# Lightning-AI/lit-llama

Hardware: NVIDIA H100
Metric: LLaMA-7B gptq.int4 decode tokens/sec (higher is better)
Workload: dtype bf16

## Files before the change

### __graft_entry__.py

```python
import os
import subprocess
import sys

ROOT = os.path.dirname(os.path.abspath(__file__))
PKG = os.path.join(ROOT, "lit-llama_b200")
CSRC = os.path.join(PKG, "csrc")
LIB = os.path.join(PKG, "libb200llama.so")
DIAG_LIB = os.path.join(ROOT, "tools", "libb200diag.so")
OBJ_DIR = os.path.join(ROOT, "build", "obj")
SOURCES = ["api.cu", "q_generic.cu", "elementwise.cu", "attention.cu", "q4_tc.cu", "q4_gemv.cu", "q4_gemv_batch.cu",
           "q8_gemv.cu", "q8_gemm.cu", "sampling.cu", "decode_mega.cu", "q4_gemm.cu", "tp_allreduce.cu", "lora.cu",
           "nll.cu", "w8_gemv_batch.cu", "q8_gemv_batch.cu"]
DIAG_SOURCES = ["microbench.cu"]
ARCH = ["-gencode", "arch=compute_90a,code=sm_90a"]
NVCC_FLAGS = ARCH + ["-O3", "-lineinfo", "-std=c++17", "-Xcompiler", "-fPIC"]


def _headers():
    return [os.path.join(CSRC, f) for f in os.listdir(CSRC) if f.endswith((".cuh", ".h"))] + \
           [os.path.join(ROOT, "include", f) for f in os.listdir(os.path.join(ROOT, "include"))]


def _compile(nvcc: str, src: str, force: bool) -> str:
    obj = os.path.join(OBJ_DIR, os.path.splitext(src)[0] + ".o")
    path = os.path.join(CSRC, src)
    if not force and os.path.exists(obj):
        t = os.path.getmtime(obj)
        if all(os.path.getmtime(d) <= t for d in [path] + _headers()):
            return obj
    cmd = [nvcc] + NVCC_FLAGS + ["-c", path, "-o", obj]
    print("[build]", " ".join(cmd), file=sys.stderr)
    subprocess.run(cmd, check=True)
    return obj


def _link(nvcc: str, objs, out: str) -> None:
    if os.path.exists(out) and all(os.path.getmtime(o) <= os.path.getmtime(out) for o in objs):
        return
    cmd = [nvcc, "-shared"] + ARCH + list(objs) + ["-o", out]
    print("[build]", " ".join(cmd), file=sys.stderr)
    subprocess.run(cmd, check=True)


def build(force: bool = False) -> None:
    from concurrent.futures import ThreadPoolExecutor

    nvcc = os.environ.get("NVCC", "/usr/local/cuda/bin/nvcc")
    os.makedirs(OBJ_DIR, exist_ok=True)
    with ThreadPoolExecutor(max_workers=min(8, os.cpu_count() or 1)) as ex:
        objs = list(ex.map(lambda s: _compile(nvcc, s, force), SOURCES + DIAG_SOURCES))
    _link(nvcc, objs[:len(SOURCES)], LIB)
    _link(nvcc, objs[len(SOURCES):], DIAG_LIB)
    _install_reference()
    if ROOT not in sys.path:
        sys.path.insert(0, ROOT)
    import lit_llama_b200
    from lit_llama_b200 import _lib

    assert _lib.lib().b2l_version() >= 100


def _install_reference(src: str = os.environ.get("LIT_LLAMA_DIR", "/root/reference")) -> None:
    import shutil
    import tempfile

    dst = os.path.join(ROOT, "oracle", "_ref")
    if os.path.isdir(os.path.join(dst, "lit_llama")) or not os.path.isfile(os.path.join(src, "pyproject.toml")):
        return
    tmp = tempfile.mkdtemp(prefix="b2l_ref_")
    try:
        work = os.path.join(tmp, "reference")
        shutil.copytree(src, work, ignore=shutil.ignore_patterns(".git", "tests", "howto"))
        cmd = [sys.executable, "-m", "pip", "install", "--no-index", "--no-build-isolation", "--no-deps", "--quiet",
               "--target", dst, work]
        print("[build]", " ".join(cmd), file=sys.stderr)
        subprocess.run(cmd, check=False)
    finally:
        shutil.rmtree(tmp, ignore_errors=True)


def smoke() -> None:
    if ROOT not in sys.path:
        sys.path.insert(0, ROOT)
    import torch

    import lit_llama_b200 as P
    from lit_llama_b200.utils import quantization
    from oracle import llama_oracle as O

    assert torch.cuda.is_available(), "smoke() needs a GPU"
    dev = torch.device("cuda", 0)
    cfg = dict(block_size=64, vocab_size=96, n_layer=2, n_head=4, n_embd=128)
    sd = O.synth_state_dict(cfg["n_layer"], cfg["n_head"], cfg["n_embd"], cfg["vocab_size"], "gptq.int4",
                            dtype=torch.bfloat16, seed=1234)
    prev = torch.get_default_dtype()
    torch.set_default_dtype(torch.bfloat16)
    try:
        with torch.device(dev), quantization("gptq.int4"):
            model = P.LLaMA(P.LLaMAConfig(**cfg))
    finally:
        torch.set_default_dtype(prev)
    model.load_state_dict(sd)
    model.eval()
    oracle = O.OracleLLaMA.from_state_dict(sd, cfg["n_layer"], cfg["n_head"], cfg["block_size"], "gptq.int4")
    prompt = torch.tensor([3, 17, 40, 41, 2, 77, 5], dtype=torch.int32)
    S = 16
    with torch.no_grad():
        got = [model(prompt.view(1, -1).to(dev), S, torch.arange(7, device=dev))]
        want = [oracle.forward(prompt.view(1, -1).long(), S, torch.arange(7))]
        for i, t in enumerate([11, 5, 90, 33]):
            got.append(model(torch.tensor([[t]], dtype=torch.int32, device=dev), S, torch.tensor([7 + i], device=dev)))
            want.append(oracle.forward(torch.tensor([[t]]), S, torch.tensor([7 + i])))
    torch.cuda.synchronize()
    for g, w in zip(got, want):
        torch.testing.assert_close(g.float().cpu(), w.float(), rtol=1e-3, atol=5e-3)
    print("smoke ok: tiny gptq.int4 prefill + 4 decode steps match the oracle", file=sys.stderr)


if __name__ == "__main__":
    build(force="--force" in sys.argv)
    if "--smoke" in sys.argv:
        smoke()
```

### include/b2l_diag.h

```cpp
#ifndef B2L_DIAG_H_
#define B2L_DIAG_H_
#include "b2l.h"
#ifdef __cplusplus
extern "C" {
#endif

const char* b2l_diag_last_error(void);

int b2l_debug_grid_flag(void* out, void* counter, int ctas_per_sm, int rounds, b2l_stream_t stream);

int b2l_debug_hmma_rate(void* out, int warps, int chains, int iters, int with_unpack, b2l_stream_t stream);

int b2l_debug_imma_rate(void* out, int warps, int chains, int iters, int n_alu, b2l_stream_t stream);

int b2l_debug_consumer_rate(void* out, int warps, int iters, int mode, int n_ctas, b2l_stream_t stream);

#ifdef __cplusplus
}
#endif
#endif
```

### lit-llama_b200/csrc/sampling.cu

```cuda
#include "b2l_common.cuh"

namespace b2l {

constexpr int SAMP_THREADS = 1024;

__device__ __forceinline__ uint32_t bf16_key(uint16_t b) {
  return (b & 0x8000u) ? (uint32_t)(uint16_t)~b : (uint32_t)(b | 0x8000u);
}

__device__ __forceinline__ void hist_add(int* hist, uint32_t bin, bool valid) {
  const uint32_t key = valid ? bin : 0xFFFFFFFFu;
  const uint32_t peers = __match_any_sync(0xffffffffu, key);
  if (valid && (threadIdx.x & 31) == __ffs(peers) - 1) atomicAdd(&hist[bin], __popc(peers));
}

__device__ __forceinline__ void find_bin(const int* hist, int want, int* sel_bin, int* sel_rank) {
  const int lane = threadIdx.x & 31;
  int c[8], s = 0;
#pragma unroll
  for (int j = 0; j < 8; ++j) { c[j] = hist[lane * 8 + j]; s += c[j]; }
  int incl = s;
#pragma unroll
  for (int o = 1; o < 32; o <<= 1) {
    const int t = __shfl_down_sync(0xffffffffu, incl, o);
    if (lane + o < 32) incl += t;
  }
  const int above = incl - s;
  if (above < want && want <= above + s) {
    int cum = above;
#pragma unroll
    for (int j = 7; j >= 0; --j) {
      if (cum + c[j] >= want) { *sel_bin = lane * 8 + j; *sel_rank = want - cum; break; }
      cum += c[j];
    }
  }
}

__device__ __forceinline__ float bits_f(uint32_t bits16) { return __uint_as_float(bits16 << 16); }

__device__ __forceinline__ uint4 load8(const __nv_bfloat16* p, int i, bool vec) {
  if (vec) return reinterpret_cast<const uint4*>(p)[i];
  const uint16_t* s = reinterpret_cast<const uint16_t*>(p) + 8 * i;
  return make_uint4(s[0] | ((uint32_t)s[1] << 16), s[2] | ((uint32_t)s[3] << 16), s[4] | ((uint32_t)s[5] << 16),
                    s[6] | ((uint32_t)s[7] << 16));
}

__global__ void __launch_bounds__(SAMP_THREADS)
    topk_softmax_kernel(const __nv_bfloat16* __restrict__ logits, long long ld, float inv_temperature, int top_k,
                        __nv_bfloat16* __restrict__ probs, const __nv_bfloat16* __restrict__ noise,
                        long long* __restrict__ token, int V) {
  extern __shared__ __align__(16) uint8_t ssm[];
  {
    const size_t row = blockIdx.x;
    logits += row * (size_t)ld;
    if (noise != nullptr) noise += row * (size_t)V;
    if (probs != nullptr) probs += row * (size_t)V;
    if (token != nullptr) token += row;
  }
  const bool vec = ((reinterpret_cast<uintptr_t>(logits) | reinterpret_cast<uintptr_t>(noise)) & 15) == 0;
  const int Vp = (V + 7) & ~7;
  uint16_t* sv = reinterpret_cast<uint16_t*>(ssm);
  uint16_t* sq = sv + Vp;
  __shared__ int hist[256];
  __shared__ int sel_hi, sel_rank, sel_lo;
  __shared__ float red[32];
  __shared__ int red_i[32];
  const int tid = threadIdx.x, lane = tid & 31, warp = tid >> 5;
  const bool select = top_k > 0 && top_k < V;
  const int nvec = V / 8;
  constexpr int PRE = 4;

  uint4 lpre[PRE], npre[PRE];
#pragma unroll
  for (int r = 0; r < PRE; ++r) {
    const int i = r * SAMP_THREADS + tid;
    lpre[r] = make_uint4(0, 0, 0, 0);
    npre[r] = make_uint4(0, 0, 0, 0);
    if (i < nvec) {
      lpre[r] = load8(logits, i, vec);
      if (noise != nullptr) npre[r] = load8(noise, i, vec);
    }
  }

  if (tid < 256) hist[tid] = 0;
  __syncthreads();
  float lmax = -INFINITY;
  const int rounds = (nvec + SAMP_THREADS - 1) / SAMP_THREADS;
#pragma unroll 1
  for (int r0 = 0; r0 < rounds; r0 += PRE) {
#pragma unroll
    for (int rr = 0; rr < PRE; ++rr) {
      const int r = r0 + rr;
      if (r >= rounds) break;
      const int i = r * SAMP_THREADS + tid;
      const bool valid = i < nvec;
      uint4 v = lpre[rr];
      if (r0 > 0) { v = make_uint4(0, 0, 0, 0); if (valid) v = load8(logits, i, vec); }
      const uint32_t w[4] = {v.x, v.y, v.z, v.w};
      uint32_t o[4];
#pragma unroll
      for (int q = 0; q < 4; ++q) {
        const float a = rbf(__uint_as_float(w[q] << 16) * inv_temperature);
        const float b = rbf(__uint_as_float(w[q] & 0xffff0000u) * inv_temperature);
        const uint32_t ab = __float_as_uint(a) >> 16, bb = __float_as_uint(b) >> 16;
        o[q] = ab | (bb << 16);
        if (valid) lmax = fmaxf(lmax, fmaxf(a, b));
        if (select) {
          hist_add(hist, bf16_key((uint16_t)ab) >> 8, valid);
          hist_add(hist, bf16_key((uint16_t)bb) >> 8, valid);
        }
      }
      if (valid) {
        reinterpret_cast<uint4*>(sv)[i] = make_uint4(o[0], o[1], o[2], o[3]);
        if (noise != nullptr) {
          uint4 n = npre[rr];
          if (r0 > 0) n = load8(noise, i, vec);
          reinterpret_cast<uint4*>(sq)[i] = n;
        }
      }
    }
  }
  {
    const int i = nvec * 8 + tid;
    const bool valid = i < V;
    uint16_t bits = 0xff80;
    if (valid) {
      const float sc = rbf(bf2f(logits[i]) * inv_temperature);
      bits = (uint16_t)(__float_as_uint(sc) >> 16);
      lmax = fmaxf(lmax, sc);
    }
    if (i < Vp) {
      sv[i] = bits;
      if (noise != nullptr) sq[i] = valid ? *reinterpret_cast<const uint16_t*>(noise + i) : (uint16_t)0x3f80;
    }
    if (select) hist_add(hist, bf16_key(bits) >> 8, valid);
  }
  lmax = warp_max(lmax);
  if (lane == 0) red[warp] = lmax;
  __syncthreads();
  float gmax = red[lane];
  gmax = warp_max(gmax);

  const int nvp = Vp / 8;
  uint32_t thr_key = 0;
  if (select) {
    if (warp == 0) find_bin(hist, top_k, &sel_hi, &sel_rank);
    __syncthreads();
    const int hi = sel_hi, rank = sel_rank;
    __syncthreads();
    if (tid < 256) hist[tid] = 0;
    __syncthreads();
    for (int base = 0; base < nvp; base += SAMP_THREADS) {
      const int i = base + tid;
      uint4 v = make_uint4(0, 0, 0, 0);
      if (i < nvp) v = reinterpret_cast<const uint4*>(sv)[i];
      const uint32_t w[4] = {v.x, v.y, v.z, v.w};
#pragma unroll
      for (int q = 0; q < 4; ++q) {
#pragma unroll
        for (int hf = 0; hf < 2; ++hf) {
          const uint32_t key = bf16_key((uint16_t)(hf ? (w[q] >> 16) : (w[q] & 0xffffu)));
          const bool hit = i < nvp && (int)(key >> 8) == hi && (8 * i + 2 * q + hf) < V;
          if (__any_sync(0xffffffffu, hit)) hist_add(hist, key & 0xFF, hit);
        }
      }
    }
    __syncthreads();
    if (warp == 0) { int dummy; find_bin(hist, rank, &sel_lo, &dummy); }
    __syncthreads();
    thr_key = ((uint32_t)hi << 8) | (uint32_t)sel_lo;
  }

  float sum = 0.f;
  for (int base = 0; base < nvp; base += SAMP_THREADS) {
    const int i = base + tid;
    if (i < nvp) {
      const uint4 v = reinterpret_cast<const uint4*>(sv)[i];
      const uint32_t w[4] = {v.x, v.y, v.z, v.w};
      bool any = false;
#pragma unroll
      for (int q = 0; q < 4; ++q)
        any = any || bf16_key((uint16_t)(w[q] & 0xffffu)) >= thr_key || bf16_key((uint16_t)(w[q] >> 16)) >= thr_key;
      if (any) {
#pragma unroll
        for (int q = 0; q < 4; ++q) {
          const uint32_t lo = w[q] & 0xffffu, hi2 = w[q] >> 16;
          if (bf16_key((uint16_t)lo) >= thr_key && lo != 0xff80u) sum += expf(bits_f(lo) - gmax);
          if (bf16_key((uint16_t)hi2) >= thr_key && hi2 != 0xff80u) sum += expf(bits_f(hi2) - gmax);
        }
      }
    }
  }
  sum = warp_sum(sum);
  __syncthreads();
  if (lane == 0) red[warp] = sum;
  __syncthreads();
  float total = red[lane];
  total = warp_sum(total);

  float best = -INFINITY;
  int best_i = 0x7fffffff;
  for (int base = 0; base < nvp; base += SAMP_THREADS) {
    const int i = base + tid;
    if (i < nvp) {
      const uint4 v = reinterpret_cast<const uint4*>(sv)[i];
      uint4 n = make_uint4(0, 0, 0, 0);
      if (noise != nullptr) n = reinterpret_cast<const uint4*>(sq)[i];
      const uint32_t w[4] = {v.x, v.y, v.z, v.w};
      const uint32_t nw[4] = {n.x, n.y, n.z, n.w};
      uint32_t o[4] = {0u, 0u, 0u, 0u};
      bool any = false;
#pragma unroll
      for (int q = 0; q < 4; ++q)
        any = any || bf16_key((uint16_t)(w[q] & 0xffffu)) >= thr_key || bf16_key((uint16_t)(w[q] >> 16)) >= thr_key;
#pragma unroll
      for (int q = 0; q < 4; ++q) {
        if (!any) break;
        uint32_t pb2[2];
#pragma unroll
        for (int hf = 0; hf < 2; ++hf) {
          const uint32_t bits = hf ? (w[q] >> 16) : (w[q] & 0xffffu);
          const bool kept = bf16_key((uint16_t)bits) >= thr_key && bits != 0xff80u;
          const float pv = kept ? expf(bits_f(bits) - gmax) / total : 0.f;
          const float pr = rbf(pv);
          pb2[hf] = __float_as_uint(pr) >> 16;
          if (noise != nullptr) {
            const int idx = 8 * i + 2 * q + hf;
            const float r = rbf(pr / bits_f(hf ? (nw[q] >> 16) : (nw[q] & 0xffffu)));
            if (idx < V && (r > best || (r == best && idx < best_i))) { best = r; best_i = idx; }
          }
        }
        o[q] = pb2[0] | (pb2[1] << 16);
      }
      if (probs != nullptr) {
        if (8 * i + 8 <= V && (reinterpret_cast<uintptr_t>(probs) & 15) == 0) {
          reinterpret_cast<uint4*>(probs)[i] = make_uint4(o[0], o[1], o[2], o[3]);
        } else {
#pragma unroll
          for (int e = 0; e < 8; ++e)
            if (8 * i + e < V) reinterpret_cast<uint16_t*>(probs)[8 * i + e] = (uint16_t)(o[e >> 1] >> (16 * (e & 1)));
        }
      }
    }
  }
  if (noise != nullptr) {
#pragma unroll
    for (int o = 16; o > 0; o >>= 1) {
      const float ob = __shfl_xor_sync(0xffffffffu, best, o);
      const int oi = __shfl_xor_sync(0xffffffffu, best_i, o);
      if (ob > best || (ob == best && oi < best_i)) { best = ob; best_i = oi; }
    }
    __syncthreads();
    if (lane == 0) { red[warp] = best; red_i[warp] = best_i; }
    __syncthreads();
    if (warp == 0) {
      best = red[lane]; best_i = red_i[lane];
#pragma unroll
      for (int o = 16; o > 0; o >>= 1) {
        const float ob = __shfl_xor_sync(0xffffffffu, best, o);
        const int oi = __shfl_xor_sync(0xffffffffu, best_i, o);
        if (ob > best || (ob == best && oi < best_i)) { best = ob; best_i = oi; }
      }
      if (lane == 0) *token = (long long)best_i;
    }
  }
}

}

using namespace b2l;

static int launch_topk(const void* logits, long long ld, float temperature, int top_k, void* probs, const void* noise, void* token,
                       int B, int V, b2l_stream_t stream, const char* who) {
  B2L_CHECK_ARG(logits && V > 0 && temperature > 0.f && top_k >= 0, "%s: bad argument", who);
  B2L_CHECK_ARG(ld == 0 || ld >= V, "%s: ld = %lld: 0 (every row reads the same logits) or at least V = %d", who, ld, V);
  B2L_CHECK_ARG(((uintptr_t)logits % 16) == 0, "%s: logits must be 16-byte aligned", who);
  B2L_CHECK_ARG(noise == nullptr || ((uintptr_t)noise % 16) == 0, "%s: noise must be 16-byte aligned", who);
  const size_t Vp = ((size_t)V + 7) & ~(size_t)7;
  const size_t smem = Vp * 2 * (noise != nullptr ? 2 : 1);
  B2L_CHECK_SUPPORTED(smem <= 200 * 1024, "%s: vocabulary %d too large for one CTA", who, V);
  static DynSmemCache smem_cache;
  if (smem > 48 * 1024)
    if (int rc = ensure_dyn_smem(topk_softmax_kernel, smem, smem_cache)) return rc;
  topk_softmax_kernel<<<B, SAMP_THREADS, smem, (cudaStream_t)stream>>>((const __nv_bfloat16*)logits, ld, 1.0f / temperature, top_k,
                                                                      (__nv_bfloat16*)probs, (const __nv_bfloat16*)noise,
                                                                      (long long*)token, V);
  B2L_LAUNCH_CHECK("topk_softmax_kernel");
  return 0;
}

extern "C" int b2l_topk_softmax(const void* logits, float temperature, int top_k, void* probs, int V, b2l_stream_t stream) {
  B2L_CHECK_ARG(probs != nullptr, "b2l_topk_softmax: null probs");
  return launch_topk(logits, V, temperature, top_k, probs, nullptr, nullptr, 1, V, stream, "b2l_topk_softmax");
}

extern "C" int b2l_topk_softmax_sample(const void* logits, float temperature, int top_k, const void* noise, void* probs,
                                       int64_t* token, int V, b2l_stream_t stream) {
  B2L_CHECK_ARG(noise != nullptr && token != nullptr, "b2l_topk_softmax_sample: null noise / token");
  return launch_topk(logits, V, temperature, top_k, probs, noise, token, 1, V, stream, "b2l_topk_softmax_sample");
}

static int check_rows(const void* logits, int B, int V, float temperature, int top_k, const char* who) {
  B2L_CHECK_ARG(logits != nullptr, "%s: null logits", who);
  B2L_CHECK_ARG(B >= 1, "%s: B = %d rows, at least 1", who, B);
  B2L_CHECK_ARG(V > 0, "%s: V = %d, at least 1", who, V);
  B2L_CHECK_ARG(temperature > 0.f, "%s: temperature %g, must be positive", who, (double)temperature);
  B2L_CHECK_ARG(top_k >= 0, "%s: top_k = %d, 0 (no filter) or positive", who, top_k);
  return 0;
}

extern "C" int b2l_topk_softmax_rows(const void* logits, int64_t ld, float temperature, int top_k, void* probs, int B, int V,
                                     b2l_stream_t stream) {
  const char* who = "b2l_topk_softmax_rows";
  if (int rc = check_rows(logits, B, V, temperature, top_k, who)) return rc;
  B2L_CHECK_ARG(probs != nullptr, "%s: null probs", who);
  return launch_topk(logits, ld, temperature, top_k, probs, nullptr, nullptr, B, V, stream, who);
}

extern "C" int b2l_topk_softmax_sample_rows(const void* logits, int64_t ld, float temperature, int top_k, const void* noise,
                                            void* probs, int64_t* tokens, int B, int V, b2l_stream_t stream) {
  const char* who = "b2l_topk_softmax_sample_rows";
  if (int rc = check_rows(logits, B, V, temperature, top_k, who)) return rc;
  B2L_CHECK_ARG(noise != nullptr, "%s: null noise", who);
  B2L_CHECK_ARG(tokens != nullptr, "%s: null tokens", who);
  return launch_topk(logits, ld, temperature, top_k, probs, noise, tokens, B, V, stream, who);
}
```

Before: 596.4.

## Split top-k softmax sampling across an 8-CTA thread-block cluster with DSMEM exchange

```diff
diff --git a/__graft_entry__.py b/__graft_entry__.py
--- a/__graft_entry__.py
+++ b/__graft_entry__.py
@@ -11,7 +11,7 @@
 SOURCES = ["api.cu", "q_generic.cu", "elementwise.cu", "attention.cu", "q4_tc.cu", "q4_gemv.cu", "q4_gemv_batch.cu",
            "q8_gemv.cu", "q8_gemm.cu", "sampling.cu", "decode_mega.cu", "q4_gemm.cu", "tp_allreduce.cu", "lora.cu",
            "nll.cu", "w8_gemv_batch.cu", "q8_gemv_batch.cu"]
-DIAG_SOURCES = ["microbench.cu"]
+DIAG_SOURCES = ["microbench.cu", "sampling_cta.cu"]
 ARCH = ["-gencode", "arch=compute_90a,code=sm_90a"]
 NVCC_FLAGS = ARCH + ["-O3", "-lineinfo", "-std=c++17", "-Xcompiler", "-fPIC"]
 
diff --git a/include/b2l_diag.h b/include/b2l_diag.h
--- a/include/b2l_diag.h
+++ b/include/b2l_diag.h
@@ -15,6 +15,9 @@
 
 int b2l_debug_consumer_rate(void* out, int warps, int iters, int mode, int n_ctas, b2l_stream_t stream);
 
+int b2l_debug_topk_softmax_cta(const void* logits, int64_t ld, float temperature, int top_k, const void* noise, void* probs,
+                               int64_t* tokens, int B, int V, b2l_stream_t stream);
+
 #ifdef __cplusplus
 }
 #endif
diff --git a/lit-llama_b200/csrc/sampling.cu b/lit-llama_b200/csrc/sampling.cu
--- a/lit-llama_b200/csrc/sampling.cu
+++ b/lit-llama_b200/csrc/sampling.cu
@@ -1,57 +1,53 @@
-#include "b2l_common.cuh"
+#include <cooperative_groups.h>
+
+#include "sampling_common.cuh"
+
+namespace cg = cooperative_groups;
 
 namespace b2l {
 
-constexpr int SAMP_THREADS = 1024;
-
-__device__ __forceinline__ uint32_t bf16_key(uint16_t b) {
-  return (b & 0x8000u) ? (uint32_t)(uint16_t)~b : (uint32_t)(b | 0x8000u);
-}
-
-__device__ __forceinline__ void hist_add(int* hist, uint32_t bin, bool valid) {
-  const uint32_t key = valid ? bin : 0xFFFFFFFFu;
-  const uint32_t peers = __match_any_sync(0xffffffffu, key);
-  if (valid && (threadIdx.x & 31) == __ffs(peers) - 1) atomicAdd(&hist[bin], __popc(peers));
-}
-
-__device__ __forceinline__ void find_bin(const int* hist, int want, int* sel_bin, int* sel_rank) {
-  const int lane = threadIdx.x & 31;
-  int c[8], s = 0;
-#pragma unroll
-  for (int j = 0; j < 8; ++j) { c[j] = hist[lane * 8 + j]; s += c[j]; }
-  int incl = s;
-#pragma unroll
-  for (int o = 1; o < 32; o <<= 1) {
-    const int t = __shfl_down_sync(0xffffffffu, incl, o);
-    if (lane + o < 32) incl += t;
-  }
-  const int above = incl - s;
-  if (above < want && want <= above + s) {
-    int cum = above;
-#pragma unroll
-    for (int j = 7; j >= 0; --j) {
-      if (cum + c[j] >= want) { *sel_bin = lane * 8 + j; *sel_rank = want - cum; break; }
-      cum += c[j];
-    }
-  }
-}
-
-__device__ __forceinline__ float bits_f(uint32_t bits16) { return __uint_as_float(bits16 << 16); }
-
-__device__ __forceinline__ uint4 load8(const __nv_bfloat16* p, int i, bool vec) {
-  if (vec) return reinterpret_cast<const uint4*>(p)[i];
-  const uint16_t* s = reinterpret_cast<const uint16_t*>(p) + 8 * i;
-  return make_uint4(s[0] | ((uint32_t)s[1] << 16), s[2] | ((uint32_t)s[3] << 16), s[4] | ((uint32_t)s[5] << 16),
-                    s[6] | ((uint32_t)s[7] << 16));
-}
-
-__global__ void __launch_bounds__(SAMP_THREADS)
-    topk_softmax_kernel(const __nv_bfloat16* __restrict__ logits, long long ld, float inv_temperature, int top_k,
-                        __nv_bfloat16* __restrict__ probs, const __nv_bfloat16* __restrict__ noise,
-                        long long* __restrict__ token, int V) {
+constexpr int SAMP_CLUSTER = 8;
+constexpr int SAMP_VT = SAMP_THREADS / SAMP_CLUSTER;
+constexpr int SAMP_CL_THREADS = 4 * SAMP_VT;
+constexpr int SAMP_CL_WARPS = SAMP_CL_THREADS / 32;
+static_assert(SAMP_VT % 32 == 0 && SAMP_CLUSTER * (SAMP_VT / 32) == 32, "the cluster holds the one-CTA kernel's 32 warps");
+static_assert(SAMP_VT / 32 == 4, "a CTA's warp sums are pushed as one 16-byte vector");
+constexpr int SAMP_HI_WORDS = 260;
+
+__device__ __forceinline__ uint32_t smem_u32(const void* p) { return (uint32_t)__cvta_generic_to_shared(p); }
+__device__ __forceinline__ uint32_t remote_u32(const void* local, int rank) {
+  uint32_t r;
+  asm volatile("mapa.shared::cluster.u32 %0, %1, %2;" : "=r"(r) : "r"(smem_u32(local)), "r"(rank));
+  return r;
+}
+__device__ __forceinline__ void st_async_v4(uint32_t dst, uint4 v, uint32_t bar) {
+  asm volatile("st.async.shared::cluster.mbarrier::complete_tx::bytes.v4.b32 [%0], {%1, %2, %3, %4}, [%5];" ::"r"(dst),
+               "r"(v.x), "r"(v.y), "r"(v.z), "r"(v.w), "r"(bar) : "memory");
+}
+__device__ __forceinline__ void st_async_v2(uint32_t dst, uint32_t a, uint32_t b, uint32_t bar) {
+  asm volatile("st.async.shared::cluster.mbarrier::complete_tx::bytes.v2.b32 [%0], {%1, %2}, [%3];" ::"r"(dst), "r"(a), "r"(b),
+               "r"(bar) : "memory");
+}
+__device__ __forceinline__ void mbar_init_expect(uint64_t* bar, uint32_t bytes) {
+  asm volatile("mbarrier.init.shared::cta.b64 [%0], 1;" ::"r"(smem_u32(bar)) : "memory");
+  asm volatile("mbarrier.arrive.expect_tx.shared::cta.b64 _, [%0], %1;" ::"r"(smem_u32(bar)), "r"(bytes) : "memory");
+}
+__device__ __forceinline__ void mbar_wait0(uint64_t* bar) {
+  asm volatile(
+      "{\n\t.reg .pred P1;\n\tLAB_WAIT:\n\t"
+      "mbarrier.try_wait.parity.shared::cta.b64 P1, [%0], 0;\n\t"
+      "@P1 bra DONE;\n\tbra LAB_WAIT;\n\tDONE:\n\t}" ::"r"(smem_u32(bar)) : "memory");
+}
+
+__global__ void __launch_bounds__(SAMP_CL_THREADS)
+    topk_softmax_cluster_kernel(const __nv_bfloat16* __restrict__ logits, long long ld, float inv_temperature, int top_k,
+                                __nv_bfloat16* __restrict__ probs, const __nv_bfloat16* __restrict__ noise,
+                                long long* __restrict__ token, int V) {
   extern __shared__ __align__(16) uint8_t ssm[];
+  cg::cluster_group cluster = cg::this_cluster();
+  const int rank = (int)cluster.block_rank();
   {
-    const size_t row = blockIdx.x;
+    const size_t row = blockIdx.x / SAMP_CLUSTER;
     logits += row * (size_t)ld;
     if (noise != nullptr) noise += row * (size_t)V;
     if (probs != nullptr) probs += row * (size_t)V;
@@ -59,40 +55,64 @@
   }
   const bool vec = ((reinterpret_cast<uintptr_t>(logits) | reinterpret_cast<uintptr_t>(noise)) & 15) == 0;
   const int Vp = (V + 7) & ~7;
+  const int nvec = V / 8;
+  const int nvp = Vp / 8;
+  const int rounds = (nvp + SAMP_THREADS - 1) / SAMP_THREADS;
+  const int nslot = rounds * SAMP_VT;
+  auto vec_of = [rank](int s) { return (s / SAMP_VT) * SAMP_THREADS + rank * SAMP_VT + s % SAMP_VT; };
   uint16_t* sv = reinterpret_cast<uint16_t*>(ssm);
-  uint16_t* sq = sv + Vp;
-  __shared__ int hist[256];
+  uint16_t* sq = sv + nslot * 8;
+  __shared__ __align__(16) int hist_hi[256];
+  __shared__ __align__(16) int hist_lo[256];
+  __shared__ __align__(16) int rx_hi[SAMP_CLUSTER][SAMP_HI_WORDS];
+  __shared__ __align__(16) int rx_lo[SAMP_CLUSTER][256];
+  __shared__ __align__(16) float wsum[32];
+  __shared__ __align__(16) float red_sum[SAMP_VT / 32];
+  __shared__ __align__(8) uint32_t cl_best[SAMP_CLUSTER][2];
+  __shared__ __align__(8) uint64_t mbar[4];
+  __shared__ int ghist[256];
   __shared__ int sel_hi, sel_rank, sel_lo;
-  __shared__ float red[32];
-  __shared__ int red_i[32];
+  __shared__ float cta_max, gmax_s;
+  __shared__ float red[SAMP_CL_WARPS];
+  __shared__ int red_i[SAMP_CL_WARPS];
   const int tid = threadIdx.x, lane = tid & 31, warp = tid >> 5;
   const bool select = top_k > 0 && top_k < V;
-  const int nvec = V / 8;
-  constexpr int PRE = 4;
+  if (tid == 0) {
+    mbar_init_expect(&mbar[0], SAMP_CLUSTER * (select ? SAMP_HI_WORDS * 4 : 16));
+    mbar_init_expect(&mbar[1], select ? SAMP_CLUSTER * 1024 : 0);
+    mbar_init_expect(&mbar[2], SAMP_CLUSTER * 16);
+    mbar_init_expect(&mbar[3], rank == 0 && noise != nullptr ? SAMP_CLUSTER * 8 : 0);
+    asm volatile("fence.mbarrier_init.release.cluster;" ::: "memory");
+  }
+  asm volatile("barrier.cluster.arrive.relaxed.aligned;" ::: "memory");
+  constexpr int PRE = 2;
 
   uint4 lpre[PRE], npre[PRE];
 #pragma unroll
   for (int r = 0; r < PRE; ++r) {
-    const int i = r * SAMP_THREADS + tid;
+    const int s = r * SAMP_CL_THREADS + tid;
+    const int i = vec_of(s);
     lpre[r] = make_uint4(0, 0, 0, 0);
     npre[r] = make_uint4(0, 0, 0, 0);
-    if (i < nvec) {
+    if (s < nslot && i < nvec) {
       lpre[r] = load8(logits, i, vec);
       if (noise != nullptr) npre[r] = load8(noise, i, vec);
     }
   }
 
-  if (tid < 256) hist[tid] = 0;
+  if (tid < 256) { hist_hi[tid] = 0; hist_lo[tid] = 0; }
   __syncthreads();
   float lmax = -INFINITY;
-  const int rounds = (nvec + SAMP_THREADS - 1) / SAMP_THREADS;
+  const int iters = (nslot + SAMP_CL_THREADS - 1) / SAMP_CL_THREADS;
 #pragma unroll 1
-  for (int r0 = 0; r0 < rounds; r0 += PRE) {
+  for (int r0 = 0; r0 < iters; r0 += PRE) {
 #pragma unroll
     for (int rr = 0; rr < PRE; ++rr) {
       const int r = r0 + rr;
-      if (r >= rounds) break;
-      const int i = r * SAMP_THREADS + tid;
+      if (r >= iters) break;
+      const int s = r * SAMP_CL_THREADS + tid;
+      if (s >= nslot) break;
+      const int i = vec_of(s);
       const bool valid = i < nvec;
       uint4 v = lpre[rr];
       if (r0 > 0) { v = make_uint4(0, 0, 0, 0); if (valid) v = load8(logits, i, vec); }
@@ -106,54 +126,79 @@
         o[q] = ab | (bb << 16);
         if (valid) lmax = fmaxf(lmax, fmaxf(a, b));
         if (select) {
-          hist_add(hist, bf16_key((uint16_t)ab) >> 8, valid);
-          hist_add(hist, bf16_key((uint16_t)bb) >> 8, valid);
+          hist_add(hist_hi, bf16_key((uint16_t)ab) >> 8, valid);
+          hist_add(hist_hi, bf16_key((uint16_t)bb) >> 8, valid);
         }
       }
       if (valid) {
-        reinterpret_cast<uint4*>(sv)[i] = make_uint4(o[0], o[1], o[2], o[3]);
+        reinterpret_cast<uint4*>(sv)[s] = make_uint4(o[0], o[1], o[2], o[3]);
         if (noise != nullptr) {
           uint4 n = npre[rr];
           if (r0 > 0) n = load8(noise, i, vec);
-          reinterpret_cast<uint4*>(sq)[i] = n;
+          reinterpret_cast<uint4*>(sq)[s] = n;
         }
       }
     }
   }
   {
+    const bool owner = nvec < nvp && (nvec % SAMP_THREADS) / SAMP_VT == rank;
+    const int s = (nvec / SAMP_THREADS) * SAMP_VT + nvec % SAMP_VT;
     const int i = nvec * 8 + tid;
-    const bool valid = i < V;
+    const bool valid = owner && i < V;
     uint16_t bits = 0xff80;
     if (valid) {
       const float sc = rbf(bf2f(logits[i]) * inv_temperature);
       bits = (uint16_t)(__float_as_uint(sc) >> 16);
       lmax = fmaxf(lmax, sc);
     }
-    if (i < Vp) {
-      sv[i] = bits;
-      if (noise != nullptr) sq[i] = valid ? *reinterpret_cast<const uint16_t*>(noise + i) : (uint16_t)0x3f80;
-    }
-    if (select) hist_add(hist, bf16_key(bits) >> 8, valid);
+    if (owner && i < Vp) {
+      sv[8 * s + tid] = bits;
+      if (noise != nullptr) sq[8 * s + tid] = valid ? *reinterpret_cast<const uint16_t*>(noise + i) : (uint16_t)0x3f80;
+    }
+    if (select) hist_add(hist_hi, bf16_key(bits) >> 8, valid);
   }
   lmax = warp_max(lmax);
   if (lane == 0) red[warp] = lmax;
   __syncthreads();
-  float gmax = red[lane];
-  gmax = warp_max(gmax);
-
-  const int nvp = Vp / 8;
+  if (warp == 0) {
+    float m = lane < SAMP_CL_WARPS ? red[lane] : -INFINITY;
+    m = warp_max(m);
+    if (lane == 0) cta_max = m;
+  }
+  __syncthreads();
+  asm volatile("barrier.cluster.wait.aligned;" ::: "memory");
+  {
+    const int nchunk = select ? SAMP_HI_WORDS / 4 : 1, c0 = select ? 0 : 64;
+    for (int j = tid; j < SAMP_CLUSTER * nchunk; j += SAMP_CL_THREADS) {
+      const int dst = j / nchunk, ch = c0 + j % nchunk;
+      const uint4 v = ch < 64 ? reinterpret_cast<const uint4*>(hist_hi)[ch] : make_uint4(__float_as_uint(cta_max), 0u, 0u, 0u);
+      st_async_v4(remote_u32(&rx_hi[rank][4 * ch], dst), v, remote_u32(&mbar[0], dst));
+    }
+  }
+  mbar_wait0(&mbar[0]);
+  if (warp == 0) {
+    float m = lane < SAMP_CLUSTER ? __int_as_float(rx_hi[lane][256]) : -INFINITY;
+    m = warp_max(m);
+    if (lane == 0) gmax_s = m;
+  }
+  if (select && tid < 256) {
+    int c = 0;
+#pragma unroll
+    for (int r = 0; r < SAMP_CLUSTER; ++r) c += rx_hi[r][tid];
+    ghist[tid] = c;
+  }
+  __syncthreads();
+  const float gmax = gmax_s;
+
   uint32_t thr_key = 0;
   if (select) {
-    if (warp == 0) find_bin(hist, top_k, &sel_hi, &sel_rank);
+    if (warp == 0) find_bin(ghist, top_k, &sel_hi, &sel_rank);
     __syncthreads();
-    const int hi = sel_hi, rank = sel_rank;
-    __syncthreads();
-    if (tid < 256) hist[tid] = 0;
-    __syncthreads();
-    for (int base = 0; base < nvp; base += SAMP_THREADS) {
-      const int i = base + tid;
+    const int hi = sel_hi, rank_in_bin = sel_rank;
+    for (int s = tid; s < nslot; s += SAMP_CL_THREADS) {
+      const int i = vec_of(s);
       uint4 v = make_uint4(0, 0, 0, 0);
-      if (i < nvp) v = reinterpret_cast<const uint4*>(sv)[i];
+      if (i < nvp) v = reinterpret_cast<const uint4*>(sv)[s];
       const uint32_t w[4] = {v.x, v.y, v.z, v.w};
 #pragma unroll
       for (int q = 0; q < 4; ++q) {
@@ -161,51 +206,66 @@
         for (int hf = 0; hf < 2; ++hf) {
           const uint32_t key = bf16_key((uint16_t)(hf ? (w[q] >> 16) : (w[q] & 0xffffu)));
           const bool hit = i < nvp && (int)(key >> 8) == hi && (8 * i + 2 * q + hf) < V;
-          if (__any_sync(0xffffffffu, hit)) hist_add(hist, key & 0xFF, hit);
+          if (__any_sync(0xffffffffu, hit)) hist_add(hist_lo, key & 0xFF, hit);
         }
       }
     }
     __syncthreads();
-    if (warp == 0) { int dummy; find_bin(hist, rank, &sel_lo, &dummy); }
+    if (tid < SAMP_CLUSTER * 64) {
+      const int dst = tid / 64, ch = tid % 64;
+      st_async_v4(remote_u32(&rx_lo[rank][4 * ch], dst), reinterpret_cast<const uint4*>(hist_lo)[ch], remote_u32(&mbar[1], dst));
+    }
+    mbar_wait0(&mbar[1]);
+    if (tid < 256) {
+      int c = 0;
+#pragma unroll
+      for (int r = 0; r < SAMP_CLUSTER; ++r) c += rx_lo[r][tid];
+      ghist[tid] = c;
+    }
+    __syncthreads();
+    if (warp == 0) { int dummy; find_bin(ghist, rank_in_bin, &sel_lo, &dummy); }
     __syncthreads();
     thr_key = ((uint32_t)hi << 8) | (uint32_t)sel_lo;
   }
 
-  float sum = 0.f;
-  for (int base = 0; base < nvp; base += SAMP_THREADS) {
-    const int i = base + tid;
-    if (i < nvp) {
-      const uint4 v = reinterpret_cast<const uint4*>(sv)[i];
-      const uint32_t w[4] = {v.x, v.y, v.z, v.w};
-      bool any = false;
-#pragma unroll
-      for (int q = 0; q < 4; ++q)
-        any = any || bf16_key((uint16_t)(w[q] & 0xffffu)) >= thr_key || bf16_key((uint16_t)(w[q] >> 16)) >= thr_key;
-      if (any) {
-#pragma unroll
-        for (int q = 0; q < 4; ++q) {
-          const uint32_t lo = w[q] & 0xffffu, hi2 = w[q] >> 16;
-          if (bf16_key((uint16_t)lo) >= thr_key && lo != 0xff80u) sum += expf(bits_f(lo) - gmax);
-          if (bf16_key((uint16_t)hi2) >= thr_key && hi2 != 0xff80u) sum += expf(bits_f(hi2) - gmax);
-        }
-      }
-    }
-  }
-  sum = warp_sum(sum);
+  if (warp < SAMP_VT / 32) {
+    float sum = 0.f;
+    for (int r = 0; r < rounds; ++r) {
+      const int i = r * SAMP_THREADS + rank * SAMP_VT + tid;
+      if (i < nvp) {
+        const uint4 v = reinterpret_cast<const uint4*>(sv)[r * SAMP_VT + tid];
+        const uint32_t w[4] = {v.x, v.y, v.z, v.w};
+        bool any = false;
+#pragma unroll
+        for (int q = 0; q < 4; ++q)
+          any = any || bf16_key((uint16_t)(w[q] & 0xffffu)) >= thr_key || bf16_key((uint16_t)(w[q] >> 16)) >= thr_key;
+        if (any) {
+#pragma unroll
+          for (int q = 0; q < 4; ++q) {
+            const uint32_t lo = w[q] & 0xffffu, hi2 = w[q] >> 16;
+            if (bf16_key((uint16_t)lo) >= thr_key && lo != 0xff80u) sum += expf(bits_f(lo) - gmax);
+            if (bf16_key((uint16_t)hi2) >= thr_key && hi2 != 0xff80u) sum += expf(bits_f(hi2) - gmax);
+          }
+        }
+      }
+    }
+    sum = warp_sum(sum);
+    if (lane == 0) red_sum[warp] = sum;
+  }
   __syncthreads();
-  if (lane == 0) red[warp] = sum;
-  __syncthreads();
-  float total = red[lane];
-  total = warp_sum(total);
+  if (tid < SAMP_CLUSTER)
+    st_async_v4(remote_u32(&wsum[rank * (SAMP_VT / 32)], tid), *reinterpret_cast<const uint4*>(red_sum), remote_u32(&mbar[2], tid));
+  mbar_wait0(&mbar[2]);
+  const float total = warp_sum(wsum[lane]);
 
   float best = -INFINITY;
   int best_i = 0x7fffffff;
-  for (int base = 0; base < nvp; base += SAMP_THREADS) {
-    const int i = base + tid;
+  for (int s = tid; s < nslot; s += SAMP_CL_THREADS) {
+    const int i = vec_of(s);
     if (i < nvp) {
-      const uint4 v = reinterpret_cast<const uint4*>(sv)[i];
+      const uint4 v = reinterpret_cast<const uint4*>(sv)[s];
       uint4 n = make_uint4(0, 0, 0, 0);
-      if (noise != nullptr) n = reinterpret_cast<const uint4*>(sq)[i];
+      if (noise != nullptr) n = reinterpret_cast<const uint4*>(sq)[s];
       const uint32_t w[4] = {v.x, v.y, v.z, v.w};
       const uint32_t nw[4] = {n.x, n.y, n.z, n.w};
       uint32_t o[4] = {0u, 0u, 0u, 0u};
@@ -250,11 +310,24 @@
       const int oi = __shfl_xor_sync(0xffffffffu, best_i, o);
       if (ob > best || (ob == best && oi < best_i)) { best = ob; best_i = oi; }
     }
-    __syncthreads();
     if (lane == 0) { red[warp] = best; red_i[warp] = best_i; }
     __syncthreads();
     if (warp == 0) {
-      best = red[lane]; best_i = red_i[lane];
+      best = lane < SAMP_CL_WARPS ? red[lane] : -INFINITY;
+      best_i = lane < SAMP_CL_WARPS ? red_i[lane] : 0x7fffffff;
+#pragma unroll
+      for (int o = 16; o > 0; o >>= 1) {
+        const float ob = __shfl_xor_sync(0xffffffffu, best, o);
+        const int oi = __shfl_xor_sync(0xffffffffu, best_i, o);
+        if (ob > best || (ob == best && oi < best_i)) { best = ob; best_i = oi; }
+      }
+      if (lane == 0)
+        st_async_v2(remote_u32(&cl_best[rank][0], 0), __float_as_uint(best), (uint32_t)best_i, remote_u32(&mbar[3], 0));
+    }
+    if (rank == 0 && warp == 0) {
+      mbar_wait0(&mbar[3]);
+      best = lane < SAMP_CLUSTER ? __uint_as_float(cl_best[lane][0]) : -INFINITY;
+      best_i = lane < SAMP_CLUSTER ? (int)cl_best[lane][1] : 0x7fffffff;
 #pragma unroll
       for (int o = 16; o > 0; o >>= 1) {
         const float ob = __shfl_xor_sync(0xffffffffu, best, o);
@@ -278,14 +351,26 @@
   B2L_CHECK_ARG(noise == nullptr || ((uintptr_t)noise % 16) == 0, "%s: noise must be 16-byte aligned", who);
   const size_t Vp = ((size_t)V + 7) & ~(size_t)7;
   const size_t smem = Vp * 2 * (noise != nullptr ? 2 : 1);
-  B2L_CHECK_SUPPORTED(smem <= 200 * 1024, "%s: vocabulary %d too large for one CTA", who, V);
+  B2L_CHECK_SUPPORTED(smem <= 200 * 1024, "%s: vocabulary %d too large", who, V);
+  const size_t cl_smem = ((Vp / 8 + SAMP_THREADS - 1) / SAMP_THREADS) * SAMP_VT * 16 * (noise != nullptr ? 2 : 1);
   static DynSmemCache smem_cache;
-  if (smem > 48 * 1024)
-    if (int rc = ensure_dyn_smem(topk_softmax_kernel, smem, smem_cache)) return rc;
-  topk_softmax_kernel<<<B, SAMP_THREADS, smem, (cudaStream_t)stream>>>((const __nv_bfloat16*)logits, ld, 1.0f / temperature, top_k,
-                                                                      (__nv_bfloat16*)probs, (const __nv_bfloat16*)noise,
-                                                                      (long long*)token, V);
-  B2L_LAUNCH_CHECK("topk_softmax_kernel");
+  if (cl_smem > 48 * 1024)
+    if (int rc = ensure_dyn_smem(topk_softmax_cluster_kernel, cl_smem, smem_cache)) return rc;  cudaLaunchConfig_t cfg = {};
+  cfg.gridDim = dim3((unsigned)B * SAMP_CLUSTER);
+  cfg.blockDim = dim3(SAMP_CL_THREADS);
+  cfg.dynamicSmemBytes = cl_smem;
+  cfg.stream = (cudaStream_t)stream;
+  cudaLaunchAttribute attr[1];
+  attr[0].id = cudaLaunchAttributeClusterDimension;
+  attr[0].val.clusterDim.x = SAMP_CLUSTER;
+  attr[0].val.clusterDim.y = 1;
+  attr[0].val.clusterDim.z = 1;
+  cfg.attrs = attr;
+  cfg.numAttrs = 1;
+  B2L_CUDA(cudaLaunchKernelEx(&cfg, topk_softmax_cluster_kernel, (const __nv_bfloat16*)logits, (long long)ld,
+                              1.0f / temperature, top_k, (__nv_bfloat16*)probs, (const __nv_bfloat16*)noise,
+                              (long long*)token, V));
+  B2L_LAUNCH_CHECK("topk_softmax_cluster_kernel");
   return 0;
 }
 
diff --git a/lit-llama_b200/csrc/sampling_common.cuh b/lit-llama_b200/csrc/sampling_common.cuh
--- /dev/null
+++ b/lit-llama_b200/csrc/sampling_common.cuh
@@ -0,0 +1,49 @@
+#pragma once
+#include "b2l_common.cuh"
+
+namespace b2l {
+
+constexpr int SAMP_THREADS = 1024;
+
+__device__ __forceinline__ uint32_t bf16_key(uint16_t b) {
+  return (b & 0x8000u) ? (uint32_t)(uint16_t)~b : (uint32_t)(b | 0x8000u);
+}
+
+__device__ __forceinline__ void hist_add(int* hist, uint32_t bin, bool valid) {
+  const uint32_t key = valid ? bin : 0xFFFFFFFFu;
+  const uint32_t peers = __match_any_sync(0xffffffffu, key);
+  if (valid && (threadIdx.x & 31) == __ffs(peers) - 1) atomicAdd(&hist[bin], __popc(peers));
+}
+
+__device__ __forceinline__ void find_bin(const int* hist, int want, int* sel_bin, int* sel_rank) {
+  const int lane = threadIdx.x & 31;
+  int c[8], s = 0;
+#pragma unroll
+  for (int j = 0; j < 8; ++j) { c[j] = hist[lane * 8 + j]; s += c[j]; }
+  int incl = s;
+#pragma unroll
+  for (int o = 1; o < 32; o <<= 1) {
+    const int t = __shfl_down_sync(0xffffffffu, incl, o);
+    if (lane + o < 32) incl += t;
+  }
+  const int above = incl - s;
+  if (above < want && want <= above + s) {
+    int cum = above;
+#pragma unroll
+    for (int j = 7; j >= 0; --j) {
+      if (cum + c[j] >= want) { *sel_bin = lane * 8 + j; *sel_rank = want - cum; break; }
+      cum += c[j];
+    }
+  }
+}
+
+__device__ __forceinline__ float bits_f(uint32_t bits16) { return __uint_as_float(bits16 << 16); }
+
+__device__ __forceinline__ uint4 load8(const __nv_bfloat16* p, int i, bool vec) {
+  if (vec) return reinterpret_cast<const uint4*>(p)[i];
+  const uint16_t* s = reinterpret_cast<const uint16_t*>(p) + 8 * i;
+  return make_uint4(s[0] | ((uint32_t)s[1] << 16), s[2] | ((uint32_t)s[3] << 16), s[4] | ((uint32_t)s[5] << 16),
+                    s[6] | ((uint32_t)s[7] << 16));
+}
+
+}
diff --git a/lit-llama_b200/csrc/sampling_cta.cu b/lit-llama_b200/csrc/sampling_cta.cu
--- /dev/null
+++ b/lit-llama_b200/csrc/sampling_cta.cu
@@ -0,0 +1,249 @@
+#include "sampling_common.cuh"
+#include "../../include/b2l_diag.h"
+
+namespace b2l {
+
+__global__ void __launch_bounds__(SAMP_THREADS)
+    topk_softmax_kernel(const __nv_bfloat16* __restrict__ logits, long long ld, float inv_temperature, int top_k,
+                        __nv_bfloat16* __restrict__ probs, const __nv_bfloat16* __restrict__ noise,
+                        long long* __restrict__ token, int V) {
+  extern __shared__ __align__(16) uint8_t ssm[];
+  {
+    const size_t row = blockIdx.x;
+    logits += row * (size_t)ld;
+    if (noise != nullptr) noise += row * (size_t)V;
+    if (probs != nullptr) probs += row * (size_t)V;
+    if (token != nullptr) token += row;
+  }
+  const bool vec = ((reinterpret_cast<uintptr_t>(logits) | reinterpret_cast<uintptr_t>(noise)) & 15) == 0;
+  const int Vp = (V + 7) & ~7;
+  uint16_t* sv = reinterpret_cast<uint16_t*>(ssm);
+  uint16_t* sq = sv + Vp;
+  __shared__ int hist[256];
+  __shared__ int sel_hi, sel_rank, sel_lo;
+  __shared__ float red[32];
+  __shared__ int red_i[32];
+  const int tid = threadIdx.x, lane = tid & 31, warp = tid >> 5;
+  const bool select = top_k > 0 && top_k < V;
+  const int nvec = V / 8;
+  constexpr int PRE = 4;
+
+  uint4 lpre[PRE], npre[PRE];
+#pragma unroll
+  for (int r = 0; r < PRE; ++r) {
+    const int i = r * SAMP_THREADS + tid;
+    lpre[r] = make_uint4(0, 0, 0, 0);
+    npre[r] = make_uint4(0, 0, 0, 0);
+    if (i < nvec) {
+      lpre[r] = load8(logits, i, vec);
+      if (noise != nullptr) npre[r] = load8(noise, i, vec);
+    }
+  }
+
+  if (tid < 256) hist[tid] = 0;
+  __syncthreads();
+  float lmax = -INFINITY;
+  const int rounds = (nvec + SAMP_THREADS - 1) / SAMP_THREADS;
+#pragma unroll 1
+  for (int r0 = 0; r0 < rounds; r0 += PRE) {
+#pragma unroll
+    for (int rr = 0; rr < PRE; ++rr) {
+      const int r = r0 + rr;
+      if (r >= rounds) break;
+      const int i = r * SAMP_THREADS + tid;
+      const bool valid = i < nvec;
+      uint4 v = lpre[rr];
+      if (r0 > 0) { v = make_uint4(0, 0, 0, 0); if (valid) v = load8(logits, i, vec); }
+      const uint32_t w[4] = {v.x, v.y, v.z, v.w};
+      uint32_t o[4];
+#pragma unroll
+      for (int q = 0; q < 4; ++q) {
+        const float a = rbf(__uint_as_float(w[q] << 16) * inv_temperature);
+        const float b = rbf(__uint_as_float(w[q] & 0xffff0000u) * inv_temperature);
+        const uint32_t ab = __float_as_uint(a) >> 16, bb = __float_as_uint(b) >> 16;
+        o[q] = ab | (bb << 16);
+        if (valid) lmax = fmaxf(lmax, fmaxf(a, b));
+        if (select) {
+          hist_add(hist, bf16_key((uint16_t)ab) >> 8, valid);
+          hist_add(hist, bf16_key((uint16_t)bb) >> 8, valid);
+        }
+      }
+      if (valid) {
+        reinterpret_cast<uint4*>(sv)[i] = make_uint4(o[0], o[1], o[2], o[3]);
+        if (noise != nullptr) {
+          uint4 n = npre[rr];
+          if (r0 > 0) n = load8(noise, i, vec);
+          reinterpret_cast<uint4*>(sq)[i] = n;
+        }
+      }
+    }
+  }
+  {
+    const int i = nvec * 8 + tid;
+    const bool valid = i < V;
+    uint16_t bits = 0xff80;
+    if (valid) {
+      const float sc = rbf(bf2f(logits[i]) * inv_temperature);
+      bits = (uint16_t)(__float_as_uint(sc) >> 16);
+      lmax = fmaxf(lmax, sc);
+    }
+    if (i < Vp) {
+      sv[i] = bits;
+      if (noise != nullptr) sq[i] = valid ? *reinterpret_cast<const uint16_t*>(noise + i) : (uint16_t)0x3f80;
+    }
+    if (select) hist_add(hist, bf16_key(bits) >> 8, valid);
+  }
+  lmax = warp_max(lmax);
+  if (lane == 0) red[warp] = lmax;
+  __syncthreads();
+  float gmax = red[lane];
+  gmax = warp_max(gmax);
+
+  const int nvp = Vp / 8;
+  uint32_t thr_key = 0;
+  if (select) {
+    if (warp == 0) find_bin(hist, top_k, &sel_hi, &sel_rank);
+    __syncthreads();
+    const int hi = sel_hi, rank = sel_rank;
+    __syncthreads();
+    if (tid < 256) hist[tid] = 0;
+    __syncthreads();
+    for (int base = 0; base < nvp; base += SAMP_THREADS) {
+      const int i = base + tid;
+      uint4 v = make_uint4(0, 0, 0, 0);
+      if (i < nvp) v = reinterpret_cast<const uint4*>(sv)[i];
+      const uint32_t w[4] = {v.x, v.y, v.z, v.w};
+#pragma unroll
+      for (int q = 0; q < 4; ++q) {
+#pragma unroll
+        for (int hf = 0; hf < 2; ++hf) {
+          const uint32_t key = bf16_key((uint16_t)(hf ? (w[q] >> 16) : (w[q] & 0xffffu)));
+          const bool hit = i < nvp && (int)(key >> 8) == hi && (8 * i + 2 * q + hf) < V;
+          if (__any_sync(0xffffffffu, hit)) hist_add(hist, key & 0xFF, hit);
+        }
+      }
+    }
+    __syncthreads();
+    if (warp == 0) { int dummy; find_bin(hist, rank, &sel_lo, &dummy); }
+    __syncthreads();
+    thr_key = ((uint32_t)hi << 8) | (uint32_t)sel_lo;
+  }
+
+  float sum = 0.f;
+  for (int base = 0; base < nvp; base += SAMP_THREADS) {
+    const int i = base + tid;
+    if (i < nvp) {
+      const uint4 v = reinterpret_cast<const uint4*>(sv)[i];
+      const uint32_t w[4] = {v.x, v.y, v.z, v.w};
+      bool any = false;
+#pragma unroll
+      for (int q = 0; q < 4; ++q)
+        any = any || bf16_key((uint16_t)(w[q] & 0xffffu)) >= thr_key || bf16_key((uint16_t)(w[q] >> 16)) >= thr_key;
+      if (any) {
+#pragma unroll
+        for (int q = 0; q < 4; ++q) {
+          const uint32_t lo = w[q] & 0xffffu, hi2 = w[q] >> 16;
+          if (bf16_key((uint16_t)lo) >= thr_key && lo != 0xff80u) sum += expf(bits_f(lo) - gmax);
+          if (bf16_key((uint16_t)hi2) >= thr_key && hi2 != 0xff80u) sum += expf(bits_f(hi2) - gmax);
+        }
+      }
+    }
+  }
+  sum = warp_sum(sum);
+  __syncthreads();
+  if (lane == 0) red[warp] = sum;
+  __syncthreads();
+  float total = red[lane];
+  total = warp_sum(total);
+
+  float best = -INFINITY;
+  int best_i = 0x7fffffff;
+  for (int base = 0; base < nvp; base += SAMP_THREADS) {
+    const int i = base + tid;
+    if (i < nvp) {
+      const uint4 v = reinterpret_cast<const uint4*>(sv)[i];
+      uint4 n = make_uint4(0, 0, 0, 0);
+      if (noise != nullptr) n = reinterpret_cast<const uint4*>(sq)[i];
+      const uint32_t w[4] = {v.x, v.y, v.z, v.w};
+      const uint32_t nw[4] = {n.x, n.y, n.z, n.w};
+      uint32_t o[4] = {0u, 0u, 0u, 0u};
+      bool any = false;
+#pragma unroll
+      for (int q = 0; q < 4; ++q)
+        any = any || bf16_key((uint16_t)(w[q] & 0xffffu)) >= thr_key || bf16_key((uint16_t)(w[q] >> 16)) >= thr_key;
+#pragma unroll
+      for (int q = 0; q < 4; ++q) {
+        if (!any) break;
+        uint32_t pb2[2];
+#pragma unroll
+        for (int hf = 0; hf < 2; ++hf) {
+          const uint32_t bits = hf ? (w[q] >> 16) : (w[q] & 0xffffu);
+          const bool kept = bf16_key((uint16_t)bits) >= thr_key && bits != 0xff80u;
+          const float pv = kept ? expf(bits_f(bits) - gmax) / total : 0.f;
+          const float pr = rbf(pv);
+          pb2[hf] = __float_as_uint(pr) >> 16;
+          if (noise != nullptr) {
+            const int idx = 8 * i + 2 * q + hf;
+            const float r = rbf(pr / bits_f(hf ? (nw[q] >> 16) : (nw[q] & 0xffffu)));
+            if (idx < V && (r > best || (r == best && idx < best_i))) { best = r; best_i = idx; }
+          }
+        }
+        o[q] = pb2[0] | (pb2[1] << 16);
+      }
+      if (probs != nullptr) {
+        if (8 * i + 8 <= V && (reinterpret_cast<uintptr_t>(probs) & 15) == 0) {
+          reinterpret_cast<uint4*>(probs)[i] = make_uint4(o[0], o[1], o[2], o[3]);
+        } else {
+#pragma unroll
+          for (int e = 0; e < 8; ++e)
+            if (8 * i + e < V) reinterpret_cast<uint16_t*>(probs)[8 * i + e] = (uint16_t)(o[e >> 1] >> (16 * (e & 1)));
+        }
+      }
+    }
+  }
+  if (noise != nullptr) {
+#pragma unroll
+    for (int o = 16; o > 0; o >>= 1) {
+      const float ob = __shfl_xor_sync(0xffffffffu, best, o);
+      const int oi = __shfl_xor_sync(0xffffffffu, best_i, o);
+      if (ob > best || (ob == best && oi < best_i)) { best = ob; best_i = oi; }
+    }
+    __syncthreads();
+    if (lane == 0) { red[warp] = best; red_i[warp] = best_i; }
+    __syncthreads();
+    if (warp == 0) {
+      best = red[lane]; best_i = red_i[lane];
+#pragma unroll
+      for (int o = 16; o > 0; o >>= 1) {
+        const float ob = __shfl_xor_sync(0xffffffffu, best, o);
+        const int oi = __shfl_xor_sync(0xffffffffu, best_i, o);
+        if (ob > best || (ob == best && oi < best_i)) { best = ob; best_i = oi; }
+      }
+      if (lane == 0) *token = (long long)best_i;
+    }
+  }
+}
+
+}
+
+using namespace b2l;
+
+extern "C" int b2l_debug_topk_softmax_cta(const void* logits, int64_t ld, float temperature, int top_k, const void* noise,
+                                          void* probs, int64_t* tokens, int B, int V, b2l_stream_t stream) {
+  B2L_CHECK_ARG(logits && B >= 1 && V > 0 && temperature > 0.f && top_k >= 0, "b2l_debug_topk_softmax_cta: bad argument");
+  B2L_CHECK_ARG(noise != nullptr || probs != nullptr, "b2l_debug_topk_softmax_cta: neither probs nor noise");
+  B2L_CHECK_ARG(noise == nullptr || tokens != nullptr, "b2l_debug_topk_softmax_cta: noise without tokens");
+  B2L_CHECK_ARG(ld == 0 || ld >= V, "b2l_debug_topk_softmax_cta: ld = %lld: 0 or at least V = %d", (long long)ld, V);
+  B2L_CHECK_ARG(((uintptr_t)logits % 16) == 0 && ((uintptr_t)noise % 16) == 0, "b2l_debug_topk_softmax_cta: logits and noise must be 16-byte aligned");
+  const size_t Vp = ((size_t)V + 7) & ~(size_t)7;
+  const size_t smem = Vp * 2 * (noise != nullptr ? 2 : 1);
+  B2L_CHECK_SUPPORTED(smem <= 200 * 1024, "b2l_debug_topk_softmax_cta: vocabulary %d too large for one CTA", V);
+  static DynSmemCache smem_cache;
+  if (smem > 48 * 1024)
+    if (int rc = ensure_dyn_smem(topk_softmax_kernel, smem, smem_cache)) return rc;
+  topk_softmax_kernel<<<B, SAMP_THREADS, smem, (cudaStream_t)stream>>>((const __nv_bfloat16*)logits, ld, 1.0f / temperature, top_k,
+                                                                      (__nv_bfloat16*)probs, (const __nv_bfloat16*)noise,
+                                                                      (long long*)tokens, V);
+  B2L_LAUNCH_CHECK("topk_softmax_kernel");
+  return 0;
+}
```

New measurement: 602.2, median of 6. Within noise of the previous version (+1.0%).
